# radhofan/Fairify

Measured on AMD Instinct MI355X. Metric: % partitions verified + partitions/sec on AC suite at 1/2/4/8 MI355X, higher is better.
Workload: dtype fp32

## Files before the change

fairify_amd/csrc/args.h:

```cpp
#pragma once
#include "common.h"

#define FA_MAX_PA 8
#define FA_MAX_RA 8
#define FA_CMAX_PA 8
#define FA_MAX_SPLIT 6

struct BoundArgs {
  const float* flat;
  const float* lo;
  const float* hi;
  const uint8_t* dead_in;
  int R;
  int symbolic;
  int G;
  int stride;
  int wstride;
  int wfloats;
  float* out_lb;
  float* out_ub;
  float* Lc; float* L0; float* Le;
  float* Uc; float* U0; float* Ue;
  float* layer_lb;
  float* layer_ub;
  uint8_t* dead_out;
  int V;
  int npa;
  int pa_idx[FA_MAX_PA];
  const float* values;
  const int* node_part;
  const uint8_t* dead_part;
  int part_mod;
  unsigned long long fold;
  const int8_t* skip_status;
  const int* skip_part;
  int skip_signdef;
  const uint8_t* row_open;
  int open_mod;
  const int8_t* phase_in;
  uint8_t* infeas;
};

#define FA_MAX_ESC 4
struct EscSteps {
  int n;
  int budget[FA_MAX_ESC];
  int open[FA_MAX_ESC];
};

struct FwdArgs {
  const float* flat;
  const float* x;
  int B;
  const uint8_t* dead;
  float* out;
  int S;
};

struct AscentArgs {
  const float* flat;
  const float* lo;
  const float* hi;
  const float* x0;
  const float* f0;
  const int* q0;
  int P, K, iters;
  int V, npa;
  int pa_idx[FA_MAX_PA];
  const int64_t* values;
  int Pp;
  const int64_t* pairs;
// ... 449 lines not shown
```

fairify_amd/csrc/audit.hip:

```cpp
#include <hip/hip_runtime.h>

#include "pointfwd.h"
#include "regfwd.h"

template <int TM>
__global__ void __launch_bounds__(FA_THREADS) __attribute__((amdgpu_waves_per_eu(TM == 10 ? 1 : 2)))
fa_audit_kernel(NetDesc net, AuditArgs a, RegNetCfg rc, PointCfg cfg) {
  extern __shared__ __attribute__((aligned(16))) float smem[];
  constexpr int XT = TM < 2 ? TM : 2;
  const int tid = threadIdx.x, lane = tid & 63, wave = tid >> 6, col = lane & 15, grp = lane >> 4;
  const int n0 = net.dims[0];
  const int V = a.V, E = a.E;
  float* slab = smem + rc.floats + wave * 32;
  uint8_t* valid = (uint8_t*)(smem + rc.floats + (FA_THREADS / 64) * 32);
  fa_stage_wperm(net, rc, a.flat, smem, tid, FA_THREADS);
  for (int i = tid; i < V * V; i += FA_THREADS) valid[i] = 0;
  __syncthreads();
  for (int q = tid; q < a.Pp; q += FA_THREADS) {
    const int64_t vi = a.pairs[2 * q], vj = a.pairs[2 * q + 1];
    if (vi >= 0 && vi < V && vj >= 0 && vj < V) valid[(int)vi * V + (int)vj] = 1;
  }
  __syncthreads();
  int8_t pslot[XT][4];
  int rstride[XT][4];
// ... 17 lines not shown
  ba.R = 16;
  ba.out_lb = slab;
  ba.out_ub = slab + 16;
  const float g0 = net.g_fwd[0];
  float Xb[XT][4], HA[TM][4], EA[TM][4], HB[TM][4], EB[TM][4];
  const int passes = (a.N + 63) / 64;
  for (int ps = blockIdx.x; ps < passes; ps += gridDim.x) {
    const int row = ps * 64 + wave * 16 + col;
    const bool rv = row < a.N;
    const int own = rv ? a.own[row] : -1;
    const bool ov = own >= 0 && own < V;
    const int oi = ov ? own : 0;
#pragma unroll
    for (int t = 0; t < XT; ++t)
#pragma unroll
      for (int i = 0; i < 4; ++i) {
        const int k = 16 * t + 4 * grp + i;
        Xb[t][i] = (k < n0 && rv) ? a.x[(size_t)row * n0 + k] : 0.f;
      }
    auto run_row = [&](int v, int e) {
#pragma unroll
      for (int t = 0; t < XT; ++t)
#pragma unroll
        for (int i = 0; i < 4; ++i) {
          float x = Xb[t][i];
          const int q = pslot[t][i];
          if (v >= 0 && q >= 0) x = (float)a.values[v * a.npa + q];
          const int rs = rstride[t][i];
          if (e >= 0 && rs > 0) x += (float)((e / rs) % base - a.tau);
          HA[t][i] = x;
          EA[t][i] = g0 * fabsf(x);
        }
      for (int l = 0; l < net.n_layers; ++l) {
        if (l & 1) fa_point_layer<TM>(net, ba, cfg, smem, l, 0, lane, HB, EB, HA, EA);
        else fa_point_layer<TM>(net, ba, cfg, smem, l, 0, lane, HA, EA, HB, EB);
      }
    };
    run_row(-1, -1);
    float lo_x = 0.f, up_x = 0.f;
    if (grp == 0) {
      lo_x = slab[col];
      up_x = slab[16 + col];
    }
    unsigned cert = 0, poss = 0;
    for (int vp = 0; vp < V; ++vp) {
      const bool vld = grp == 0 && ov && valid[oi * V + vp] != 0;
      for (int e = 0; e < E; ++e) {
        if (__ballot(vld && !((cert >> vp) & 1u)) == 0) break;
        run_row(vp, e);
        if (vld) {
          const float lp = slab[col], up = slab[16 + col];
          if ((up_x < 0.f && lp > 0.f) || (lo_x > 0.f && up < 0.f)) cert |= 1u << vp;
          if ((lo_x < 0.f && up > 0.f) || (up_x > 0.f && lp < 0.f)) poss |= 1u << vp;
        }
      }
    }
    if (grp == 0 && rv) {
      a.cert[row] = ov ? (int)cert : 0;
      a.poss[row] = ov ? (int)poss : 0;
      a.own_sign[row] = (int8_t)(!ov ? 0 : up_x < 0.f ? -1 : lo_x > 0.f ? 1 : 0);
    }
  }
}

namespace {
typedef void (*AuditKernel)(NetDesc, AuditArgs, RegNetCfg, PointCfg);
AuditKernel select_audit(int TM) {
  if (TM <= 1) return fa_audit_kernel<1>;
// ... 38 lines not shown
```

fairify_amd/csrc/bab_runtime.cpp:

```cpp
#include <hip/hip_runtime.h>
#include <pybind11/numpy.h>
#include <pybind11/pybind11.h>
#include <pybind11/stl.h>

#include <algorithm>
#include <chrono>
#include <cmath>
#include <cstring>
#include <stdexcept>
#include <utility>
#include <vector>

#include "runtime_host.h"

namespace py = pybind11;

extern "C" int fa_certify_launch(CertArgs a, hipStream_t stream);
extern "C" int fa_split_launch(SplitArgs a, hipStream_t stream);
extern "C" int fa_mark_unknown_launch(const int* part, int n, int8_t* status, hipStream_t stream);
extern "C" int fa_settle_launch(SettleArgs s, hipStream_t stream);
extern "C" int fa_crown_launch(const NetDesc& net, BoundArgs a, hipStream_t stream);
extern "C" int fa_refine_launch(const NetDesc& net, BoundArgs a, hipStream_t stream);
extern "C" int fa_backward_launch(const NetDesc& net, BoundArgs a, hipStream_t stream);
extern "C" int fa_refine_crown_launch(const NetDesc& net, BoundArgs a, hipStream_t stream);
// ... 9 lines not shown
using fa_rt::ck;
using fa_rt::ckl;

bool point_skip_closed() {
  static const bool v = [] {
    const char* e = getenv("FAIRIFY_POINT_SKIP_CLOSED");
    return !(e && e[0] == '0');
  }();
  return v;
}

bool cert_skip_closed() {
  static const bool v = [] {
    const char* e = getenv("FAIRIFY_CERT_SKIP_CLOSED");
    return !(e && e[0] == '0');
  }();
  return v;
}

bool fuse_settle() {
  static const bool v = [] {
    const char* e = getenv("FAIRIFY_FUSE_SETTLE");
    return e && e[0] == '1';
  }();
  return v;
}

bool skip_signdef() {
  static const bool v = [] {
    const char* e = getenv("FAIRIFY_REFINE_SKIP_SIGNDEF");
    return !(e && e[0] == '0');
  }();
  return v;
}

}

class BabRuntime {
 public:
  BabRuntime(py::handle net, uintptr_t flat, std::vector<int> pa, std::vector<float> values_f,
             std::vector<int64_t> values_i, std::vector<int64_t> pairs, std::vector<int> ra, float tau,
             std::vector<uint8_t> shared, int capacity, int batch_nodes, int cand_cap, double unit, bool crown,
             int split_target, int refine, bool smear, py::object keep)
      : net_(fa_net_desc(net)),
        flat_((const float*)flat),
        keep_(std::move(keep)),
        pa_(std::move(pa)),
        ra_(std::move(ra)),
        tau_(tau),
        cap_(capacity),
        batch_(batch_nodes),
        cand_cap_(cand_cap),
        unit_(unit),
        crown_(crown),
        refine_(crown ? refine : 0),
        smear_(smear),
        split_target_(std::max(2, split_target)),
        sink_(net_.dims[0]) {
    n0_ = net_.dims[0];
    npa_ = (int)pa_.size();
    if (npa_ == 0 || npa_ > FA_CMAX_PA || (int)ra_.size() > FA_MAX_RA) throw std::invalid_argument("bad PA/RA");
    V_ = (int)(values_i.size() / npa_);
    Pp_ = (int)(pairs.size() / 2);
    relaxed_ = !ra_.empty() && tau_ > 0;
    norient_ = relaxed_ ? 2 : 1;
    if ((int)shared.size() != n0_) throw std::invalid_argument("shared mask size");
    vals_f_.ensure(values_f.size());
    vals_i_.ensure(values_i.size());
    pairs_.ensure(pairs.size());
    shared_.ensure(shared.size());
    ck(hipMemcpy(vals_f_.p, values_f.data(), values_f.size() * sizeof(float), hipMemcpyHostToDevice), "cp");
    ck(hipMemcpy(vals_i_.p, values_i.data(), values_i.size() * sizeof(int64_t), hipMemcpyHostToDevice), "cp");
    ck(hipMemcpy(pairs_.p, pairs.data(), pairs.size() * sizeof(int64_t), hipMemcpyHostToDevice), "cp");
    ck(hipMemcpy(shared_.p, shared.data(), shared.size(), hipMemcpyHostToDevice), "cp");
    pool_[0] = pool_[1] = 0;
    const size_t R = (size_t)batch_ * V_;
    for (int s = 0; s < (relaxed_ ? 2 : 1); ++s) form_[s].ensure(R, n0_, net_.n_neurons, crown_ || smear_);
    const size_t Q = (size_t)Pp_ * norient_;
    gmin_.ensure(batch_ * Q);
    tstar_.ensure(batch_ * Q);
    open_.ensure(batch_);
    leaf_.ensure(batch_);
    score_.ensure(batch_);
    split_.ensure(batch_);
    cv_.ensure(batch_);
    co_.ensure(batch_);
    cand_.ensure((size_t)2 * batch_ * n0_);
    scores_.ensure((size_t)batch_ * 2 * n0_);
    pe_lb_.ensure(2 * (size_t)batch_);
    pe_ub_.ensure(2 * (size_t)batch_);
    sink_.ensure_cand(cand_cap_, kCandFloor);
    counters_.ensure(5);
// ... 118 lines not shown
        const float* bphi = relaxed_ ? phi_[cur].p + (size_t)s * n0_ : bhi;
        const int* bpart = part_[cur].p + s;
        launch_bounds(blo, bhi, bpart, nb, 0, dead_part, st);
        if (relaxed_) launch_bounds(bplo, bphi, bpart, nb, 1, dead_part, st);
        const int sx = relaxed_ ? 1 : 0;
        CertArgs c{};
        c.Nn = nb; c.n0 = n0_; c.V = V_; c.Pp = Pp_; c.norient = norient_;
        const fa_rt::FormBufs &fx = form_[0], &fp = form_[sx];
        c.Lc = fx.Lc.p; c.L0 = fx.L0.p; c.Le = fx.Le.p; c.Uc = fx.Uc.p; c.U0 = fx.U0.p; c.Ue = fx.Ue.p;
        c.Lcp = fp.Lc.p; c.L0p = fp.L0.p; c.Lep = fp.Le.p; c.Ucp = fp.Uc.p; c.U0p = fp.U0.p; c.Uep = fp.Ue.p;
        c.olb = fx.olb.p; c.oub = fx.oub.p; c.olbp = fp.olb.p; c.oubp = fp.oub.p;
        c.xlo = blo; c.xhi = bhi; c.xplo = bplo; c.xphi = bphi;
        c.pairs = pairs_.p; c.values = vals_i_.p; c.npa = npa_;
        for (int k = 0; k < npa_; ++k) c.pa_idx[k] = pa_[k];
        c.nra = relaxed_ ? (int)ra_.size() : 0;
        for (int k = 0; k < c.nra; ++k) c.ra_idx[k] = ra_[k];
        c.tau = tau_;
        c.shared = shared_.p;
        c.unit = (float)unit_;
        c.gmarg = fa_rt::gamma_up(2 * n0_ + 4, unit_);
        c.gmin = gmin_.p; c.tstar = tstar_.p;
        c.open = open_.p; c.score = score_.p; c.split_dim = split_.p;
        c.cand_x = cand_.p; c.cand_xp = cand_.p + (size_t)nb * n0_;
        c.cand_v = cv_.p; c.cand_o = co_.p;
        c.scores = scores_.p; c.leaf = leaf_.p;
        if (cert_skip_closed()) { c.skip_closed = 1; c.status = status_.p; c.part = bpart; }
        if (smear_ && !relaxed_) {
          c.smear = 1;
          c.lay_lb = fx.lay_lb.p; c.lay_ub = fx.lay_ub.p; c.lay_N = net_.n_neurons;
          c.W0T = w0t_.p; c.n1 = net_.dims[1];
        }
        ckl(fa_certify_launch(c, st), "certify");
        fa_rt::screen_points(net_, flat_, cand_.p, 2 * nb, pe_lb_.p, pe_ub_.p, st, bpart, nb,
                             (const uint8_t*)dead_part, point_skip_closed() ? open_.p : nullptr, nb);
        SplitArgs sa{};
        sa.Nn = nb; sa.n0 = n0_; sa.relaxed = relaxed_ ? 1 : 0; sa.nra = relaxed_ ? (int)ra_.size() : 0;
        for (int k = 0; k < sa.nra; ++k) sa.ra_idx[k] = ra_[k];
        sa.V = V_; sa.Pp = Pp_; sa.norient = norient_; sa.tau = tau_;
        sa.xlo = blo; sa.xhi = bhi; sa.xplo = bplo; sa.xphi = bphi; sa.part = bpart;
        sa.open = open_.p; sa.leaf = leaf_.p; sa.scores = scores_.p;
        sa.cand_x = c.cand_x; sa.cand_xp = c.cand_xp; sa.pe_lb = pe_lb_.p; sa.pe_ub = pe_ub_.p;
        sa.olb = c.olb; sa.oub = c.oub; sa.olbp = c.olbp; sa.oubp = c.oubp;
        sa.pairs = pairs_.p; sa.values = vals_i_.p; sa.npa = npa_;
        for (int k = 0; k < npa_; ++k) sa.pa_idx[k] = pa_[k];
        sa.shared = shared_.p;
        sa.status = status_.p; sa.part_nodes = nodes_.p; sa.part_open = open_left_.p; sa.lvl_open = lvl_open_.p;
        sa.nodes_start = nodes_start_.p;
        sa.prev_start = prev_start_.p;
        sa.budget = budget; sa.m = FA_MAX_SPLIT; sa.target = split_target_;
        sa.pbudget = inline_esc ? pbudget_.p : nullptr;
        sa.prob = inline_esc ? prob_.p : nullptr;
        sa.budget2 = budget2;
        sa.oxlo = lo_[nxt].p; sa.oxhi = hi_[nxt].p;
        sa.oxplo = relaxed_ ? plo_[nxt].p : nullptr; sa.oxphi = relaxed_ ? phi_[nxt].p : nullptr;
        sa.opart = part_[nxt].p; sa.count_out = cnt; sa.cap = pool_[nxt];
        sa.cand_buf = sink_.records(); sa.cand_count = cnt + 1; sa.cand_cap = sink_.cand_alloc_;
        if (s + nb >= n_in && fuse_settle_) {
          sa.settle = se;
          settled = true;
        }
        ckl(fa_split_launch(sa, st), "split");
        launches += (relaxed_ ? 2 : 1) * (refine_ == 2 ? 1 : 2) + 3;
      }
      if (!settled) {
        ckl(fa_settle_launch(se, st), "settle");
        ++launches;
      }
// ... 86 lines not shown
      if (rc == -1) crown_ = false;
      else ckl(rc, "crown");
    }
  }

  void ensure_pool(int i, long long need) {
    const int want = (int)std::min<long long>(std::max<long long>(need, 1), cap_);
    if (want <= pool_[i]) return;
    const int n = fa_rt::grow_to(pool_[i], want, 1 << 16, cap_);
    const size_t cn = (size_t)n * n0_;
    lo_[i].ensure(cn);
    hi_[i].ensure(cn);
    part_[i].ensure(n);
    if (relaxed_) {
      plo_[i].ensure(cn);
      phi_[i].ensure(cn);
    }
    pool_[i] = n;
  }

  NetDesc net_;
  const float* flat_;
  py::object keep_;
  fa_exact::ExactChecker exact_;
  std::vector<int> pa_, ra_;
  float tau_;
  int cap_, batch_, cand_cap_;
  static constexpr int kCandFloor = 1 << 16;
  int pool_[2] = {0, 0};
  double unit_;
  bool crown_ = false;
  int refine_ = 0;
  bool smear_ = false;
  bool fuse_settle_ = fuse_settle();
  int split_target_ = 256;
  int n0_ = 0, npa_ = 0, V_ = 0, Pp_ = 0, norient_ = 1;
  bool relaxed_ = false;
  DevBuf<float> vals_f_, w0t_;
  DevBuf<int64_t> vals_i_, pairs_;
  DevBuf<uint8_t> shared_;
  DevBuf<float> lo_[2], hi_[2], plo_[2], phi_[2];
  DevBuf<int> part_[2];
  fa_rt::FormBufs form_[2];
  DevBuf<float> gmin_, tstar_, score_, cand_, scores_, pe_lb_, pe_ub_;
  DevBuf<uint8_t> open_, leaf_;
  DevBuf<int64_t> split_, cv_, co_;
  DevBuf<int> counters_, nodes_, open_left_, lvl_open_, nodes_start_, prev_start_, out_, pbudget_;
  DevBuf<int8_t> status_;
  DevBuf<uint8_t> prob_;
  DevBuf<unsigned char> stage_;
  fa_rt::LevelCounters hcount_;
  fa_mem::HostBuf hstage_, hout_;
  fa_rt::CandSink sink_;
};

void register_bab(py::module& m) {
  py::class_<BabRuntime>(m, "BabRuntime")
      .def(py::init<py::handle, uintptr_t, std::vector<int>, std::vector<float>, std::vector<int64_t>,
                    std::vector<int64_t>, std::vector<int>, float, std::vector<uint8_t>, int, int, int, double, bool,
                    int, int, bool, py::object>(),
           py::arg("net"), py::arg("flat"), py::arg("pa"), py::arg("values_f"), py::arg("values_i"),
           py::arg("pairs"), py::arg("ra"), py::arg("tau"), py::arg("shared"), py::arg("capacity"),
           py::arg("batch_nodes"), py::arg("cand_cap"), py::arg("unit"), py::arg("crown") = true,
           py::arg("split_target") = 256, py::arg("refine") = 0, py::arg("smear") = false, py::arg("keep") = py::none())
      .def("set_fuse_settle", &BabRuntime::set_fuse_settle, py::arg("on"))
      .def("solve", &BabRuntime::solve, py::arg("lo"), py::arg("hi"), py::arg("status"), py::arg("budget"),
// ... 5 lines not shown
```

fairify_amd/csrc/bindings.cpp:

```cpp
#include <hip/hip_runtime.h>
#include <pybind11/pybind11.h>
#include <pybind11/stl.h>

#include <algorithm>
#include <cmath>
#include <cstring>
#include <cstdint>
#include <stdexcept>
#include <vector>

#include "kwargs.h"
#include "runtime_host.h"

extern "C" int fa_bounds_launch(const NetDesc& net, BoundArgs args, hipStream_t stream);
extern "C" int fa_crown_phase_launch(const NetDesc& net, CrownPhaseArgs a, hipStream_t stream);
extern "C" size_t fa_crown_phase_bytes(const NetDesc& net);
extern "C" int fa_point_try_launch(const NetDesc& net, BoundArgs a, hipStream_t stream);
extern "C" int fa_forward_launch(const NetDesc& net, FwdArgs a, hipStream_t stream);
extern "C" int fa_sim_launch(const NetDesc& net, SimArgs a, hipStream_t stream);
extern "C" int fa_sim_shaped(const NetDesc& net);
extern "C" int fa_sym_shaped(const NetDesc& net, unsigned long long fold_mask);
extern "C" int fa_sym_geometry(const NetDesc& net, unsigned long long fold_mask, int* out);
extern "C" int fa_crown_shaped(const NetDesc& net, int mask);
extern "C" int fa_refine_shaped(const NetDesc& net, int logit);
// ... 318 lines not shown
    ckl(fa_crown_launch(net.d, a, finish(k)), "crown");
  });

  m.def("refine", [](const Net& net, py::kwargs kw) {
    Kw k("refine", kw);
    BoundArgs a = bound_args(k, LAYERS);
    a.phase_in = k.ptr<const int8_t>("phase_in");
    a.infeas = k.ptr<uint8_t>("infeas");
    const int rc = fa_refine_launch(net.d, a, finish(k));
    if (rc < -1) throw std::runtime_error("refine launch failed, code " + std::to_string(rc));
    return rc;
  });
  m.def("refine_crown", [](const Net& net, py::kwargs kw) {
    Kw k("refine_crown", kw);
    const BoundArgs a = bound_args(k, OUT | FORMS | LAYERS);
    const int rc = fa_refine_crown_launch(net.d, a, finish(k));
    if (rc < -1) throw std::runtime_error("refine_crown launch failed, code " + std::to_string(rc));
    return rc;
  });
  m.def("backward_bounds", [](const Net& net, py::kwargs kw) {
    Kw k("backward_bounds", kw);
    const BoundArgs a = bound_args(k, OUT | FORMS);
    const int rc = fa_backward_launch(net.d, a, finish(k));
    if (rc < -1) throw std::runtime_error("backward_bounds launch failed, code " + std::to_string(rc));
    return rc;
  });

  m.def("point_bounds", [](const Net& net, py::kwargs kw) {
    Kw k("point_bounds", kw);
    BoundArgs a = bound_args(k, OUT, "x", "x");
    a.row_open = k.ptr<const uint8_t>("row_open");
    a.open_mod = k.i("open_mod", 0);
    if (a.row_open && a.open_mod <= 0) throw std::invalid_argument("point_bounds: row_open needs open_mod > 0");
    const hipStream_t stream = finish(k);
    const int rc = fa_point_try_launch(net.d, a, stream);
    if (rc < 0) ckl(-rc, "point_bounds");
    if (rc == 0) ckl(fa_bounds_launch(net.d, a, stream), "point_bounds(ibp)");
  });

  m.def("forward", [](const Net& net, uintptr_t flat, uintptr_t x, int B, uintptr_t dead, uintptr_t out,
                      uintptr_t stream) {
    FwdArgs a{};
    a.flat = P<const float>(flat);
    a.x = P<const float>(x);
    a.B = B;
    a.dead = P<const uint8_t>(dead);
    a.out = P<float>(out);
    ckl(fa_forward_launch(net.d, a, (hipStream_t)stream), "forward");
  });

  m.def("sim", [](const Net& net, py::kwargs kw) {
    Kw k("sim", kw);
    SimArgs a{};
    fill_query(a, k, "too many PA/RA dims");
    fill_samples(a, k, "too many PA/RA dims");
    a.counts = k.need<int>("counts");
    a.found = k.need<uint8_t>("found");
    a.wit_x = k.need<float>("wit_x");
    a.wit_xp = k.need<float>("wit_xp");
    a.z0 = k.ptr<float>("z0");
    a.keys = k.ptr<int>("keys");
    a.split = k.i("split");
    a.regcount = k.i("regcount");
    if (a.split < 1 || (a.split > 1 && !a.keys)) throw std::invalid_argument("sim: split > 1 needs a keys buffer");
    ckl(fa_sim_launch(net.d, a, finish(k)), "sim");
  });
// ... 462 lines not shown
```

fairify_amd/csrc/count.hip:

```cpp
#include <hip/hip_runtime.h>

#include "pointfwd.h"
#include "regfwd.h"
#include "wave.h"

template <int TM>
__global__ void __launch_bounds__(FA_THREADS) __attribute__((amdgpu_waves_per_eu(TM == 7 ? 2 : 1)))
fa_count_enum_kernel(NetDesc net, EnumArgs a, RegNetCfg rc, PointCfg cfg) {
  extern __shared__ __attribute__((aligned(16))) float smem[];
  constexpr int XT = TM < 2 ? TM : 2;
  const int tid = threadIdx.x, lane = tid & 63, wave = tid >> 6, col = lane & 15, grp = lane >> 4;
  const int n0 = net.dims[0];
  const int V = a.V, E = a.E;
  const bool rx = a.nra > 0;
  float* slab = smem + rc.floats + wave * (V + 1) * 32;
  float* s_lo = smem + rc.floats + (FA_THREADS / 64) * (V + 1) * 32;
  int* s_w = (int*)(s_lo + n0);
  int* s_st = s_w + n0;
  int* cnt = s_st + n0;
  uint8_t* valid = (uint8_t*)(cnt + 2);
  fa_stage_wperm(net, rc, a.flat, smem, tid, FA_THREADS);
  for (int i = tid; i < V * V; i += FA_THREADS) valid[i] = 0;
  __syncthreads();
  for (int q = tid; q < a.Pp; q += FA_THREADS) {
// ... 41 lines not shown
      cnt[0] = 0;
      cnt[1] = ok ? (int)vol : 0;
      if (!ok) a.cert[leaf] = -1;
    }
    __syncthreads();
    const int vol = cnt[1];
    int ncert = 0;
    for (int s0 = 0; s0 < vol; s0 += FA_THREADS / 4) {
      const int s = s0 + wave * 16 + col;
      const bool sv = s < vol;
#pragma unroll
      for (int t = 0; t < XT; ++t)
#pragma unroll
        for (int i = 0; i < 4; ++i) {
          const int k = 16 * t + 4 * grp + i;
          Xb[t][i] = (k < n0 && sv) ? s_lo[k] + (float)((s / s_st[k]) % s_w[k]) : 0.f;
        }
      auto run_row = [&](int v, int e, int r) {
#pragma unroll
        for (int t = 0; t < XT; ++t)
#pragma unroll
          for (int i = 0; i < 4; ++i) {
            float x = Xb[t][i];
            const int q = pslot[t][i];
            if (q >= 0) x = (float)a.values[v * a.npa + q];
            const int rs = rstride[t][i];
            if (e >= 0 && rs > 0) x += (float)((e / rs) % base - a.tau);
            HA[t][i] = x;
            EA[t][i] = g0 * fabsf(x);
          }
        ba.out_lb = slab + r * 32;
        ba.out_ub = slab + r * 32 + 16;
        for (int l = 0; l < net.n_layers; ++l) {
          if (l & 1) fa_point_layer<TM>(net, ba, cfg, smem, l, 0, lane, HB, EB, HA, EA);
          else fa_point_layer<TM>(net, ba, cfg, smem, l, 0, lane, HA, EA, HB, EB);
        }
      };
      for (int v = 0; v < V; ++v) run_row(v, -1, v);
      bool cert = false, poss = false;
      auto test_row = [&](int vp, int r) {
        const float lp = slab[r * 32 + col], up = slab[r * 32 + 16 + col];
        for (int v = 0; v < V; ++v) {
          if (!valid[v * V + vp]) continue;
          const float lv = slab[v * 32 + col], uv = slab[v * 32 + 16 + col];
          cert = cert || (uv < 0.f && lp > 0.f) || (lv > 0.f && up < 0.f);
          poss = poss || (lv < 0.f && up > 0.f) || (uv > 0.f && lp < 0.f);
        }
      };
      if (!rx) {
        if (grp == 0)
          for (int vp = 0; vp < V; ++vp) test_row(vp, vp);
      } else {
        for (int e = 0; e < E; ++e)
          for (int vp = 0; vp < V; ++vp) {
            run_row(vp, e, V);
            if (grp == 0) test_row(vp, V);
          }
      }
      if (grp == 0 && sv) {
        if (cert) {
          ++ncert;
        } else if (poss) {
          const int slot = atomicAdd(&a.amb[leaf], 1);
          if (slot < FA_RATE_SLOTS) a.amb_idx[(size_t)leaf * FA_RATE_SLOTS + slot] = s;
        }
      }
    }
    ncert += __shfl_xor(ncert, 1);
// ... 185 lines not shown
```

fairify_amd/csrc/pointfwd.h:

```cpp
#pragma once
#include "args.h"

struct PointCfg {
  int w_lds[FA_MAX_LAYERS];
  int b_lds[FA_MAX_LAYERS];
  int bp_lds[FA_MAX_LAYERS];
};

template <int TM>
__device__ __forceinline__ void fa_point_layer(const NetDesc& net, const BoundArgs& a, const PointCfg& cfg,
                                               const float* smem, int l, int p0, int lane,
                                               const float (&H)[TM][4], const float (&E)[TM][4],
                                               float (&H2)[TM][4], float (&E2)[TM][4]) {
  const int col = lane & 15, grp = lane >> 4;
  const int n_in = net.dims[l], n_out = net.dims[l + 1];
  const int tin = (n_in + 15) >> 4, tout = (n_out + 15) >> 4;
  const float* sw = smem + cfg.w_lds[l];
  const float* sbp = smem + cfg.bp_lds[l];
  const bool last = l == net.n_layers - 1;
  const float gg = net.g_fwd[l];
  const float gi = net.g_one;
  const float gnext = last ? 0.f : net.g_fwd[l + 1];
  const int noff = net.neuron_off[l];
  const int p = p0 + col;
  const bool pv = p < a.R;
  const bool masked = !last && (a.dead_in || a.dead_part);
  const uint8_t* drow = nullptr;
  if (masked && pv) {
    if (a.dead_in) drow = a.dead_in + (size_t)p * net.n_hidden + noff;
    else drow = a.dead_part + (size_t)a.node_part[a.part_mod ? p % a.part_mod : p] * net.n_hidden + noff;
  }
#pragma unroll
  for (int jt = 0; jt < TM; ++jt) {
    if (jt >= tout) break;
    const float4 b4 = *reinterpret_cast<const float4*>(sbp + 16 * jt + 4 * grp);
    const float bl[4] = {b4.x, b4.y, b4.z, b4.w};
    bool forced[4] = {false, false, false, false};
    if (masked) {
#pragma unroll
      for (int i = 0; i < 4; ++i) {
        const int j = 16 * jt + 4 * grp + i;
        forced[i] = drow && j < n_out && drow[j] != 0;
      }
    }
    f32x4 Z = {0.f, 0.f, 0.f, 0.f}, Q = {0.f, 0.f, 0.f, 0.f};
    const float4* wq = reinterpret_cast<const float4*>(sw) + (size_t)jt * tin * 64 + lane;
#pragma unroll
    for (int t = 0; t < TM; ++t) {
      if (t >= tin) break;
      const float4 w4 = wq[t * 64];
      const float wv[4] = {w4.x, w4.y, w4.z, w4.w};
#pragma unroll
      for (int i = 0; i < 4; ++i) {
        Z = fa_mfma4(wv[i], H[t][i], Z);
        Q = fa_mfma4(fabsf(wv[i]), E[t][i], Q);
      }
    }
#pragma unroll
    for (int i = 0; i < 4; ++i) {
      const int j = 16 * jt + 4 * grp + i;
      const bool jv = j < n_out;
      const float b = bl[i];
      const float z = Z[i] + b;
      const float d = fmaf(gi, fabsf(z), fmaf(Q[i], 1.f + 2.f * gg, gg * fabsf(b)));
      if (last) {
        if (j == 0 && pv) {
          a.out_lb[p] = z - d;
          a.out_ub[p] = z + d;
        }
        continue;
      }
      const bool zero = !jv || forced[i] || (z + d <= 0.f);
      const float h = zero ? 0.f : fmaxf(z, 0.f);
      const float e = zero ? 0.f : d;
      H2[jt][i] = h;
      E2[jt][i] = fmaf(gnext, h, e);
    }
  }
}
```

fairify_amd/csrc/points.hip:

```cpp
#include <hip/hip_runtime.h>

#include "launch.h"
#include "pointfwd.h"

template <int TM>
__global__ void __launch_bounds__(FA_THREADS) __attribute__((amdgpu_waves_per_eu(TM == 7 ? 2 : 1))) fa_point_kernel(NetDesc net, BoundArgs a, PointCfg cfg) {
  extern __shared__ __attribute__((aligned(16))) float smem[];
  const int tid = threadIdx.x;
  if (a.row_open) {
    const int nw = FA_THREADS / 64;
    const int ntile = (a.R + 15) >> 4;
    int any = 0;
    for (int tile = blockIdx.x * nw + (tid >> 6); tile < ntile; tile += gridDim.x * nw) {
      const int p = tile * 16 + (tid & 15);
      any |= p < a.R && a.row_open[p % a.open_mod];
    }
    if (!__syncthreads_or(any)) return;
  }
  {
    const float4* src = reinterpret_cast<const float4*>(a.flat + net.wperm_off);
    float4* dst = reinterpret_cast<float4*>(smem);
    for (int e = tid; e < (net.wperm_floats >> 2); e += FA_THREADS) dst[e] = src[e];
    for (int l = 0; l < net.n_layers; ++l) {
      const int n_out = net.dims[l + 1];
      const float* b = a.flat + net.wperm_off + cfg.b_lds[l];
      for (int j = tid; j < ((n_out + 15) & ~15); j += FA_THREADS) smem[cfg.bp_lds[l] + j] = j < n_out ? b[j] : 0.f;
    }
  }
  __syncthreads();
  const int lane = tid & 63, col = lane & 15, grp = lane >> 4;
  const int wave = tid >> 6, nw = FA_THREADS / 64;
  const int n0 = net.dims[0];
  const int tin0 = (n0 + 15) >> 4;
  const float g0 = net.g_fwd[0];
  const int ntile = (a.R + 15) >> 4;
  for (int tile = blockIdx.x * nw + wave; tile < ntile; tile += gridDim.x * nw) {
    const int p0 = tile * 16;
    const int p = p0 + col;
    if (a.row_open && !__any(p < a.R && a.row_open[p % a.open_mod])) continue;
    float HA[TM][4], EA[TM][4], HB[TM][4], EB[TM][4];
#pragma unroll
    for (int t = 0; t < TM; ++t) {
      if (t >= tin0) break;
#pragma unroll
      for (int i = 0; i < 4; ++i) {
        const int k = 16 * t + 4 * grp + i;
        const float x = (k < n0 && p < a.R) ? a.lo[(size_t)p * n0 + k] : 0.f;
        HA[t][i] = x;
        EA[t][i] = g0 * fabsf(x);
      }
    }
    for (int l = 0; l < net.n_layers; ++l) {
      if (l & 1) fa_point_layer<TM>(net, a, cfg, smem, l, p0, lane, HB, EB, HA, EA);
      else fa_point_layer<TM>(net, a, cfg, smem, l, p0, lane, HA, EA, HB, EB);
    }
  }
}

namespace {
typedef void (*PointKernel)(NetDesc, BoundArgs, PointCfg);

#define FA_POINT_TMS(X) X(1) X(2) X(4) X(7) X(10)

PointKernel select_point(int TM) {
  switch (fa_tm_bucket(TM)) {
#define FA_POINT_CASE(T) \
  case T: return fa_point_kernel<T>;
    FA_POINT_TMS(FA_POINT_CASE)
#undef FA_POINT_CASE
    default: return nullptr;
  }
}
}

extern "C" int fa_point_try_launch(const NetDesc& net, BoundArgs a, hipStream_t stream) {
  if (a.R <= 0) return 1;
  PointKernel k = select_point(fa_widest_tiles(net, 0, net.n_layers));
  if (!k) return 0;
  PointCfg cfg{};
  int off = fa_lay_weights(net, net.n_layers, cfg.w_lds, 0);
  off = fa_lay_biases(net, net.n_layers, cfg.b_lds, off);
  if (((off + 3) & ~3) != net.wperm_floats) return -1;
  if ((size_t)net.wperm_floats * sizeof(float) > 150 * 1024) return 0;
  off = net.wperm_floats;
  for (int l = 0; l < net.n_layers; ++l) {
    cfg.bp_lds[l] = off;
    off += fa_tiles(net.dims[l + 1]) * 16;
// ... 17 lines not shown
```

fairify_amd/csrc/rate.hip:

```cpp
#include <hip/hip_runtime.h>

#include "pointfwd.h"
#include "regfwd.h"

#ifndef FA_RATE_WPE7
#define FA_RATE_WPE7 2
#endif

template <int TM>
__global__ void __launch_bounds__(FA_THREADS) __attribute__((amdgpu_waves_per_eu(TM == 7 ? FA_RATE_WPE7 : 1)))
fa_rate_kernel(NetDesc net, RateArgs a, RegNetCfg rc, PointCfg cfg) {
  extern __shared__ __attribute__((aligned(16))) float smem[];
  constexpr int XT = TM < 2 ? TM : 2;
  const int tid = threadIdx.x, lane = tid & 63, wave = tid >> 6, col = lane & 15, grp = lane >> 4;
  const int n0 = net.dims[0];
  const int G = a.split;
  const int p = blockIdx.x / G;
  const int g = blockIdx.x - p * G;
  const int V = a.V, E = a.E;
  const bool rx = a.nra > 0;
  const int64_t pid = a.pids[p];
  float* slab = smem + rc.floats + wave * (V + 1) * 32;
  float* s_lo = smem + rc.floats + (FA_THREADS / 64) * (V + 1) * 32;
  float* s_hi = s_lo + n0;
// ... 31 lines not shown
      rstride[t][i] = rs;
    }
  BoundArgs ba{};
  ba.R = 16;
  const float g0 = net.g_fwd[0];
  float Xb[XT][4], HA[TM][4], EA[TM][4], HB[TM][4], EB[TM][4];
  int ncert = 0;
  for (int s0 = g * 64; s0 < a.n_samples; s0 += G * 64) {
    const int s = s0 + wave * 16 + col;
    const bool sv = s < a.n_samples;
#pragma unroll
    for (int t = 0; t < XT; ++t)
#pragma unroll
      for (int i = 0; i < 4; ++i) {
        const int k = 16 * t + 4 * grp + i;
        Xb[t][i] = (k < n0 && sv) ? fa_sample_coord(a.seed, pid, s, k, s_lo[k], s_hi[k]) : 0.f;
      }
    auto run_row = [&](int v, int e, int r) {
#pragma unroll
      for (int t = 0; t < XT; ++t)
#pragma unroll
        for (int i = 0; i < 4; ++i) {
          float x = Xb[t][i];
          const int q = pslot[t][i];
          if (q >= 0) x = (float)a.values[v * a.npa + q];
          const int rs = rstride[t][i];
          if (e >= 0 && rs > 0) x += (float)((e / rs) % base - a.tau);
          HA[t][i] = x;
          EA[t][i] = g0 * fabsf(x);
        }
      ba.out_lb = slab + r * 32;
      ba.out_ub = slab + r * 32 + 16;
      for (int l = 0; l < net.n_layers; ++l) {
        if (l & 1) fa_point_layer<TM>(net, ba, cfg, smem, l, 0, lane, HB, EB, HA, EA);
        else fa_point_layer<TM>(net, ba, cfg, smem, l, 0, lane, HA, EA, HB, EB);
      }
    };
    for (int v = 0; v < V; ++v) run_row(v, -1, v);
    bool cert = false, poss = false;
    auto test_row = [&](int vp, int r) {
      const float lp = slab[r * 32 + col], up = slab[r * 32 + 16 + col];
      for (int v = 0; v < V; ++v) {
        if (!valid[v * V + vp]) continue;
        const float lv = slab[v * 32 + col], uv = slab[v * 32 + 16 + col];
        cert = cert || (uv < 0.f && lp > 0.f) || (lv > 0.f && up < 0.f);
        poss = poss || (lv < 0.f && up > 0.f) || (uv > 0.f && lp < 0.f);
      }
    };
    if (!rx) {
      if (grp == 0)
        for (int vp = 0; vp < V; ++vp) test_row(vp, vp);
    } else {
      for (int e = 0; e < E; ++e)
        for (int vp = 0; vp < V; ++vp) {
          run_row(vp, e, V);
          if (grp == 0) test_row(vp, V);
        }
    }
    if (grp == 0 && sv) {
      if (cert) {
        ++ncert;
      } else if (poss) {
        const int slot = atomicAdd(&a.amb[p], 1);
        if (slot < FA_RATE_SLOTS) a.amb_idx[(size_t)p * FA_RATE_SLOTS + slot] = s;
      }
    }
  }
  ncert += __shfl_xor(ncert, 1);
// ... 56 lines not shown
```

fairify_amd/csrc/runtime_host.h:

```cpp
#pragma once

#include <hip/hip_runtime.h>
#include <pybind11/numpy.h>
#include <pybind11/pybind11.h>

#include <algorithm>
#include <cmath>
#include <cstring>
#include <stdexcept>
#include <string>
#include <vector>

#include "args.h"
#include "devmem.h"
#include "exact_host.h"

extern "C" int fa_bounds_launch(const NetDesc& net, BoundArgs args, hipStream_t stream);
extern "C" int fa_point_try_launch(const NetDesc& net, BoundArgs a, hipStream_t stream);
extern "C" int fa_set_status_launch(const int* idx, int n, int8_t* status, int8_t v, hipStream_t stream);

namespace fa_rt {

namespace py = pybind11;

// ... 36 lines not shown
  return e;
}

struct LevelCounters {
  fa_mem::HostBuf hcount_buf_{true};
  LevelCounters() { hcount_buf_.ensure(4 * sizeof(int)); }
  void reset() { std::memset(hcount_buf_.p, 0, 4 * sizeof(int)); }
  int* host_ptr() { return reinterpret_cast<int*>(hcount_buf_.p); }
  int children() const { return reinterpret_cast<volatile const int*>(hcount_buf_.p)[0]; }
  int candidates() const { return reinterpret_cast<volatile const int*>(hcount_buf_.p)[1]; }
};

struct FormBufs {
  fa_mem::DevBuf<float> Lc, L0, Le, Uc, U0, Ue, olb, oub, lay_lb, lay_ub;
  void ensure(size_t rows, int n0, int n_neurons, bool with_layers) {
    Lc.ensure(rows * n0); Uc.ensure(rows * n0);
    L0.ensure(rows); Le.ensure(rows); U0.ensure(rows); Ue.ensure(rows);
    olb.ensure(rows); oub.ensure(rows);
    if (with_layers) { lay_lb.ensure(rows * n_neurons); lay_ub.ensure(rows * n_neurons); }
  }
  void fill(BoundArgs& b) const {
    b.out_lb = olb.p; b.out_ub = oub.p;
    b.Lc = Lc.p; b.L0 = L0.p; b.Le = Le.p; b.Uc = Uc.p; b.U0 = U0.p; b.Ue = Ue.p;
  }
  void fill(CrownPhaseArgs& c) const {
    c.out_lb = olb.p; c.out_ub = oub.p;
    c.Lc = Lc.p; c.L0 = L0.p; c.Le = Le.p; c.Uc = Uc.p; c.U0 = U0.p; c.Ue = Ue.p;
    c.layer_lb = lay_lb.p; c.layer_ub = lay_ub.p;
  }
};

inline void screen_points(const NetDesc& net, const float* flat, const float* pts, int rows, float* lb, float* ub,
                          hipStream_t st, const int* node_part = nullptr, int part_mod = 0,
                          const uint8_t* dead_part = nullptr, const uint8_t* row_open = nullptr, int open_mod = 0) {
  BoundArgs b{};
  b.flat = flat; b.lo = pts; b.hi = pts; b.R = rows; b.symbolic = 0;
  b.out_lb = lb; b.out_ub = ub;
  if (dead_part) { b.node_part = node_part; b.part_mod = part_mod; b.dead_part = dead_part; }
  if (row_open) { b.row_open = row_open; b.open_mod = open_mod; }
  const int prc = fa_point_try_launch(net, b, st);
  if (prc < 0) ckl(-prc, "points");
  if (prc == 0) ckl(fa_bounds_launch(net, b, st), "bounds(points)");
}

struct CandSink {
  static constexpr int kMax = 1 << 24;
  fa_mem::HostBuf cand_host_{true};
  fa_mem::HostBuf hidx_;
  fa_mem::DevBuf<int> idx_;
  int cand_alloc_ = 0;
  const int n0_;
  explicit CandSink(int n0) : n0_(n0) {}

  float* records() { return reinterpret_cast<float*>(cand_host_.p); }

  void ensure_cand(long long need, int floor) {
    if (need <= cand_alloc_) return;
    const int n = grow_to(cand_alloc_, (int)std::min<long long>(need, kMax), floor, kMax);
    cand_host_.ensure((size_t)n * (2 * n0_ + 1) * sizeof(float));
    cand_alloc_ = n;
  }

  void confirm_candidates(int n_cand, fa_exact::Witnesses& w, const fa_exact::ExactChecker* chk, py::object& confirm,
                          int8_t* status, hipStream_t st) {
    const size_t w2 = (size_t)2 * n0_;
    const std::vector<float> rec(records(), records() + (size_t)n_cand * (w2 + 1));
    const std::vector<int> newly = fa_exact::select_witnesses(
        rec.data(), n_cand, w, chk,
        [&](const std::vector<int>& slots, const std::vector<float>& pairs, const std::vector<int>& parts) {
          py::gil_scoped_acquire gil;
          const int na = (int)slots.size();
          py::array_t<float> abuf({na, 2 * n0_});
// ... 18 lines not shown
```

fairify_amd/csrc/wave.h:

```cpp
#pragma once
#include <hip/hip_runtime.h>

__device__ __forceinline__ float fa_gam(int k, float u) {
#pragma clang fp contract(off)
  const float ku = (float)(k + 2) * u;
  return ku / (1.f - ku) * (1.f + 4.f * u);
}

template <int G>
__device__ __forceinline__ float fa_group_sum(float v) {
#pragma unroll
  for (int off = G / 2; off > 0; off >>= 1) v += __shfl_xor(v, off, 64);
  return v;
}

template <int G>
__device__ __forceinline__ void fa_group_argmax(float& s, int& i) {
#pragma unroll
  for (int off = G / 2; off > 0; off >>= 1) {
    const float s2 = __shfl_xor(s, off, 64);
    const int i2 = __shfl_xor(i, off, 64);
    if (s2 > s || (s2 == s && i2 < i)) { s = s2; i = i2; }
  }
}

__device__ __forceinline__ int fa_wave_incl_scan(int v, int lane) {
#pragma unroll
  for (int o = 1; o < 64; o <<= 1) {
    const int u = __shfl_up(v, o);
    if (lane >= o) v += u;
  }
  return v;
}
```

Before: 300,300.

## Compact open rows per wave in point screening and prefetch weights

The point-bound kernel can now gather only the open (not yet closed) rows from a 64-row window, using a ballot and an nth-set-bit lookup. Waves then process dense 16-row tiles of live rows, so fewer tiles are wasted on mostly-closed rows. This path is enabled only when the widest layer spans 3 to 7 sixteen-wide tiles, and an env var can turn it off. The layer routine also changes to take a per-lane row index, prefetch the next weight float4 behind a sched barrier, load the dead mask branchlessly, and run the last-layer output path before the ReLU handling. Risks are extra ballot/popcount overhead and a changed tile-to-wave mapping.

```diff
diff --git a/fairify_amd/csrc/args.h b/fairify_amd/csrc/args.h
--- a/fairify_amd/csrc/args.h
+++ b/fairify_amd/csrc/args.h
@@ -37,6 +37,7 @@
   int skip_signdef;
   const uint8_t* row_open;
   int open_mod;
+  int row_gather;
   const int8_t* phase_in;
   uint8_t* infeas;
 };
diff --git a/fairify_amd/csrc/audit.hip b/fairify_amd/csrc/audit.hip
--- a/fairify_amd/csrc/audit.hip
+++ b/fairify_amd/csrc/audit.hip
@@ -73,8 +73,8 @@
           EA[t][i] = g0 * fabsf(x);
         }
       for (int l = 0; l < net.n_layers; ++l) {
-        if (l & 1) fa_point_layer<TM>(net, ba, cfg, smem, l, 0, lane, HB, EB, HA, EA);
-        else fa_point_layer<TM>(net, ba, cfg, smem, l, 0, lane, HA, EA, HB, EB);
+        if (l & 1) fa_point_layer<TM>(net, ba, cfg, smem, l, lane & 15, true, lane, HB, EB, HA, EA);
+        else fa_point_layer<TM>(net, ba, cfg, smem, l, lane & 15, true, lane, HA, EA, HB, EB);
       }
     };
     run_row(-1, -1);
diff --git a/fairify_amd/csrc/bab_runtime.cpp b/fairify_amd/csrc/bab_runtime.cpp
--- a/fairify_amd/csrc/bab_runtime.cpp
+++ b/fairify_amd/csrc/bab_runtime.cpp
@@ -65,6 +65,11 @@
     return !(e && e[0] == '0');
   }();
   return v;
+}
+
+bool env_on(const char* name) {
+  const char* e = getenv(name);
+  return !(e && e[0] == '0');
 }
 
 }
@@ -91,6 +96,11 @@
         split_target_(std::max(2, split_target)),
         sink_(net_.dims[0]) {
     n0_ = net_.dims[0];
+    {
+      int wide = 1;
+      for (int l = 0; l <= net_.n_layers; ++l) wide = std::max(wide, (net_.dims[l] + 15) / 16);
+      point_gather_ = wide >= 3 && wide <= 7;
+    }
     npa_ = (int)pa_.size();
     if (npa_ == 0 || npa_ > FA_CMAX_PA || (int)ra_.size() > FA_MAX_RA) throw std::invalid_argument("bad PA/RA");
     V_ = (int)(values_i.size() / npa_);
@@ -275,7 +285,8 @@
         }
         ckl(fa_certify_launch(c, st), "certify");
         fa_rt::screen_points(net_, flat_, cand_.p, 2 * nb, pe_lb_.p, pe_ub_.p, st, bpart, nb,
-                             (const uint8_t*)dead_part, point_skip_closed() ? open_.p : nullptr, nb);
+                             (const uint8_t*)dead_part, point_skip_closed() ? open_.p : nullptr, nb,
+                             point_gather_ && env_on("FAIRIFY_POINT_GATHER") ? 1 : 0);
         SplitArgs sa{};
         sa.Nn = nb; sa.n0 = n0_; sa.relaxed = relaxed_ ? 1 : 0; sa.nra = relaxed_ ? (int)ra_.size() : 0;
         for (int k = 0; k < sa.nra; ++k) sa.ra_idx[k] = ra_[k];
@@ -428,6 +439,7 @@
   bool crown_ = false;
   int refine_ = 0;
   bool smear_ = false;
+  bool point_gather_ = false;
   bool fuse_settle_ = fuse_settle();
   int split_target_ = 256;
   int n0_ = 0, npa_ = 0, V_ = 0, Pp_ = 0, norient_ = 1;
diff --git a/fairify_amd/csrc/bindings.cpp b/fairify_amd/csrc/bindings.cpp
--- a/fairify_amd/csrc/bindings.cpp
+++ b/fairify_amd/csrc/bindings.cpp
@@ -374,6 +374,11 @@
     a.row_open = k.ptr<const uint8_t>("row_open");
     a.open_mod = k.i("open_mod", 0);
     if (a.row_open && a.open_mod <= 0) throw std::invalid_argument("point_bounds: row_open needs open_mod > 0");
+    a.row_gather = k.i("row_gather", 0);
+    a.dead_part = k.ptr<const uint8_t>("dead_part");
+    a.node_part = k.ptr<const int>("node_part");
+    a.part_mod = k.i("part_mod", 0);
+    if (a.dead_part && !a.node_part) throw std::invalid_argument("point_bounds: dead_part without node_part");
     const hipStream_t stream = finish(k);
     const int rc = fa_point_try_launch(net.d, a, stream);
     if (rc < 0) ckl(-rc, "point_bounds");
diff --git a/fairify_amd/csrc/count.hip b/fairify_amd/csrc/count.hip
--- a/fairify_amd/csrc/count.hip
+++ b/fairify_amd/csrc/count.hip
@@ -97,8 +97,8 @@
         ba.out_lb = slab + r * 32;
         ba.out_ub = slab + r * 32 + 16;
         for (int l = 0; l < net.n_layers; ++l) {
-          if (l & 1) fa_point_layer<TM>(net, ba, cfg, smem, l, 0, lane, HB, EB, HA, EA);
-          else fa_point_layer<TM>(net, ba, cfg, smem, l, 0, lane, HA, EA, HB, EB);
+          if (l & 1) fa_point_layer<TM>(net, ba, cfg, smem, l, lane & 15, true, lane, HB, EB, HA, EA);
+          else fa_point_layer<TM>(net, ba, cfg, smem, l, lane & 15, true, lane, HA, EA, HB, EB);
         }
       };
       for (int v = 0; v < V; ++v) run_row(v, -1, v);
diff --git a/fairify_amd/csrc/pointfwd.h b/fairify_amd/csrc/pointfwd.h
--- a/fairify_amd/csrc/pointfwd.h
+++ b/fairify_amd/csrc/pointfwd.h
@@ -9,10 +9,10 @@
 
 template <int TM>
 __device__ __forceinline__ void fa_point_layer(const NetDesc& net, const BoundArgs& a, const PointCfg& cfg,
-                                               const float* smem, int l, int p0, int lane,
+                                               const float* smem, int l, int p, bool pv, int lane,
                                                const float (&H)[TM][4], const float (&E)[TM][4],
                                                float (&H2)[TM][4], float (&E2)[TM][4]) {
-  const int col = lane & 15, grp = lane >> 4;
+  const int grp = lane >> 4;
   const int n_in = net.dims[l], n_out = net.dims[l + 1];
   const int tin = (n_in + 15) >> 4, tout = (n_out + 15) >> 4;
   const float* sw = smem + cfg.w_lds[l];
@@ -22,57 +22,63 @@
   const float gi = net.g_one;
   const float gnext = last ? 0.f : net.g_fwd[l + 1];
   const int noff = net.neuron_off[l];
-  const int p = p0 + col;
-  const bool pv = p < a.R;
   const bool masked = !last && (a.dead_in || a.dead_part);
   const uint8_t* drow = nullptr;
-  if (masked && pv) {
-    if (a.dead_in) drow = a.dead_in + (size_t)p * net.n_hidden + noff;
-    else drow = a.dead_part + (size_t)a.node_part[a.part_mod ? p % a.part_mod : p] * net.n_hidden + noff;
+  if (masked) {
+    const int pc = p < a.R ? p : a.R - 1;
+    if (a.dead_in) drow = a.dead_in + (size_t)pc * net.n_hidden + noff;
+    else drow = a.dead_part + (size_t)a.node_part[a.part_mod ? pc % a.part_mod : pc] * net.n_hidden + noff;
   }
 #pragma unroll
   for (int jt = 0; jt < TM; ++jt) {
     if (jt >= tout) break;
     const float4 b4 = *reinterpret_cast<const float4*>(sbp + 16 * jt + 4 * grp);
     const float bl[4] = {b4.x, b4.y, b4.z, b4.w};
-    bool forced[4] = {false, false, false, false};
+    uint8_t fb[4] = {0, 0, 0, 0};
     if (masked) {
 #pragma unroll
       for (int i = 0; i < 4; ++i) {
         const int j = 16 * jt + 4 * grp + i;
-        forced[i] = drow && j < n_out && drow[j] != 0;
+        fb[i] = drow[j < n_out ? j : 0];
       }
     }
     f32x4 Z = {0.f, 0.f, 0.f, 0.f}, Q = {0.f, 0.f, 0.f, 0.f};
     const float4* wq = reinterpret_cast<const float4*>(sw) + (size_t)jt * tin * 64 + lane;
+    f32x4 wn = *reinterpret_cast<const f32x4*>(wq);
 #pragma unroll
     for (int t = 0; t < TM; ++t) {
       if (t >= tin) break;
-      const float4 w4 = wq[t * 64];
-      const float wv[4] = {w4.x, w4.y, w4.z, w4.w};
+      const f32x4 w4 = wn;
+      if (t + 1 < TM) wn = *reinterpret_cast<const f32x4*>(wq + (t + 1 < tin ? t + 1 : tin - 1) * 64);
+      __builtin_amdgcn_sched_barrier(0);
+      const float wv[4] = {w4[0], w4[1], w4[2], w4[3]};
 #pragma unroll
       for (int i = 0; i < 4; ++i) {
         Z = fa_mfma4(wv[i], H[t][i], Z);
         Q = fa_mfma4(fabsf(wv[i]), E[t][i], Q);
       }
     }
+    asm volatile("" ::"v"(wn));
+    float zz[4], dd[4];
+#pragma unroll
+    for (int i = 0; i < 4; ++i) {
+      const float b = bl[i];
+      zz[i] = Z[i] + b;
+      dd[i] = fmaf(gi, fabsf(zz[i]), fmaf(Q[i], 1.f + 2.f * gg, gg * fabsf(b)));
+    }
+    if (last) {
+      if (jt == 0 && grp == 0 && pv) {
+        a.out_lb[p] = zz[0] - dd[0];
+        a.out_ub[p] = zz[0] + dd[0];
+      }
+      continue;
+    }
 #pragma unroll
     for (int i = 0; i < 4; ++i) {
       const int j = 16 * jt + 4 * grp + i;
-      const bool jv = j < n_out;
-      const float b = bl[i];
-      const float z = Z[i] + b;
-      const float d = fmaf(gi, fabsf(z), fmaf(Q[i], 1.f + 2.f * gg, gg * fabsf(b)));
-      if (last) {
-        if (j == 0 && pv) {
-          a.out_lb[p] = z - d;
-          a.out_ub[p] = z + d;
-        }
-        continue;
-      }
-      const bool zero = !jv || forced[i] || (z + d <= 0.f);
-      const float h = zero ? 0.f : fmaxf(z, 0.f);
-      const float e = zero ? 0.f : d;
+      const bool zero = (j >= n_out) | (fb[i] != 0) | (zz[i] + dd[i] <= 0.f);
+      const float h = zero ? 0.f : fmaxf(zz[i], 0.f);
+      const float e = zero ? 0.f : dd[i];
       H2[jt][i] = h;
       E2[jt][i] = fmaf(gnext, h, e);
     }
diff --git a/fairify_amd/csrc/points.hip b/fairify_amd/csrc/points.hip
--- a/fairify_amd/csrc/points.hip
+++ b/fairify_amd/csrc/points.hip
@@ -2,11 +2,13 @@
 
 #include "launch.h"
 #include "pointfwd.h"
+#include "wave.h"
 
 template <int TM>
 __global__ void __launch_bounds__(FA_THREADS) __attribute__((amdgpu_waves_per_eu(TM == 7 ? 2 : 1))) fa_point_kernel(NetDesc net, BoundArgs a, PointCfg cfg) {
   extern __shared__ __attribute__((aligned(16))) float smem[];
   const int tid = threadIdx.x;
+  const bool gather = a.row_open && a.row_gather;
   if (a.row_open) {
     const int nw = FA_THREADS / 64;
     const int ntile = (a.R + 15) >> 4;
@@ -34,10 +36,24 @@
   const int tin0 = (n0 + 15) >> 4;
   const float g0 = net.g_fwd[0];
   const int ntile = (a.R + 15) >> 4;
-  for (int tile = blockIdx.x * nw + wave; tile < ntile; tile += gridDim.x * nw) {
+  int it = 0;
+  for (int tile = blockIdx.x * nw + wave; tile - wave < ntile; tile += gridDim.x * nw, ++it) {
     const int p0 = tile * 16;
-    const int p = p0 + col;
-    if (a.row_open && !__any(p < a.R && a.row_open[p % a.open_mod])) continue;
+    int p = p0 + col;
+    bool pv = p < a.R;
+    if (gather) {
+      const int s0 = (tile - wave) * 16;
+      const int ps = s0 + lane;
+      const unsigned long long live = __ballot(ps < a.R && a.row_open[ps % a.open_mod]);
+      const int nlive = __popcll(live);
+      const int base = 16 * ((wave - it) & (nw - 1));
+      if (base >= nlive) continue;
+      p = s0 + fa_gather_row(live, nlive, base + col);
+      pv = base + col < nlive;
+    } else {
+      if (tile >= ntile) break;
+      if (a.row_open && !__any(pv && a.row_open[p % a.open_mod])) continue;
+    }
     float HA[TM][4], EA[TM][4], HB[TM][4], EB[TM][4];
 #pragma unroll
     for (int t = 0; t < TM; ++t) {
@@ -51,8 +67,8 @@
       }
     }
     for (int l = 0; l < net.n_layers; ++l) {
-      if (l & 1) fa_point_layer<TM>(net, a, cfg, smem, l, p0, lane, HB, EB, HA, EA);
-      else fa_point_layer<TM>(net, a, cfg, smem, l, p0, lane, HA, EA, HB, EB);
+      if (l & 1) fa_point_layer<TM>(net, a, cfg, smem, l, p, pv, lane, HB, EB, HA, EA);
+      else fa_point_layer<TM>(net, a, cfg, smem, l, p, pv, lane, HA, EA, HB, EB);
     }
   }
 }
diff --git a/fairify_amd/csrc/rate.hip b/fairify_amd/csrc/rate.hip
--- a/fairify_amd/csrc/rate.hip
+++ b/fairify_amd/csrc/rate.hip
@@ -87,8 +87,8 @@
       ba.out_lb = slab + r * 32;
       ba.out_ub = slab + r * 32 + 16;
       for (int l = 0; l < net.n_layers; ++l) {
-        if (l & 1) fa_point_layer<TM>(net, ba, cfg, smem, l, 0, lane, HB, EB, HA, EA);
-        else fa_point_layer<TM>(net, ba, cfg, smem, l, 0, lane, HA, EA, HB, EB);
+        if (l & 1) fa_point_layer<TM>(net, ba, cfg, smem, l, lane & 15, true, lane, HB, EB, HA, EA);
+        else fa_point_layer<TM>(net, ba, cfg, smem, l, lane & 15, true, lane, HA, EA, HB, EB);
       }
     };
     for (int v = 0; v < V; ++v) run_row(v, -1, v);
diff --git a/fairify_amd/csrc/runtime_host.h b/fairify_amd/csrc/runtime_host.h
--- a/fairify_amd/csrc/runtime_host.h
+++ b/fairify_amd/csrc/runtime_host.h
@@ -92,12 +92,13 @@
 
 inline void screen_points(const NetDesc& net, const float* flat, const float* pts, int rows, float* lb, float* ub,
                           hipStream_t st, const int* node_part = nullptr, int part_mod = 0,
-                          const uint8_t* dead_part = nullptr, const uint8_t* row_open = nullptr, int open_mod = 0) {
+                          const uint8_t* dead_part = nullptr, const uint8_t* row_open = nullptr, int open_mod = 0,
+                          int row_gather = 0) {
   BoundArgs b{};
   b.flat = flat; b.lo = pts; b.hi = pts; b.R = rows; b.symbolic = 0;
   b.out_lb = lb; b.out_ub = ub;
   if (dead_part) { b.node_part = node_part; b.part_mod = part_mod; b.dead_part = dead_part; }
-  if (row_open) { b.row_open = row_open; b.open_mod = open_mod; }
+  if (row_open) { b.row_open = row_open; b.open_mod = open_mod; b.row_gather = row_gather; }
   const int prc = fa_point_try_launch(net, b, st);
   if (prc < 0) ckl(-prc, "points");
   if (prc == 0) ckl(fa_bounds_launch(net, b, st), "bounds(points)");
diff --git a/fairify_amd/csrc/wave.h b/fairify_amd/csrc/wave.h
--- a/fairify_amd/csrc/wave.h
+++ b/fairify_amd/csrc/wave.h
@@ -24,6 +24,23 @@
   }
 }
 
+__device__ __forceinline__ int fa_nth_set_bit(unsigned long long mask, int k) {
+  int pos = 0;
+#pragma unroll
+  for (int w = 32; w > 0; w >>= 1) {
+    const int c = __popcll((mask >> pos) & ((1ull << w) - 1ull));
+    if (k >= c) {
+      k -= c;
+      pos += w;
+    }
+  }
+  return pos;
+}
+
+__device__ __forceinline__ int fa_gather_row(unsigned long long live, int nlive, int k) {
+  return fa_nth_set_bit(live, k < nlive ? k : nlive - 1);
+}
+
 __device__ __forceinline__ int fa_wave_incl_scan(int v, int lane) {
 #pragma unroll
   for (int o = 1; o < 64; o <<= 1) {
```

Result: no change. 300,900 (median of 3 runs) (+0.2%).
